# VISION-SJTU/UniDefense

Measured on AMD Instinct MI355X. Metric: images/sec fwd+bwd (256x256, EffNet-b4), higher is better.
Workload: dtype f32

## Files before the change

### include/unidefense_hip.h

```cpp
#ifndef UNIDEFENSE_HIP_H
#define UNIDEFENSE_HIP_H
#include <stdint.h>

#ifdef __cplusplus
extern "C" {
#endif

#define UD_EINVAL (-1000)

typedef void* ud_stream_t;

typedef struct {
    int N, Hin, Win, Cin, Hout, Wout, KH, KW, stride, pad_t, pad_l, transposed;
} ud_conv_geom;

typedef struct {
    const float* A; const float* B; float* C;
    int M, N, K;
    long lda, ldb, ldc;
    int a_mode, b_mode, out_mode, split_k;
    int batch; long strideA, strideB, strideC;
    ud_conv_geom g;
    double* stat_sum; double* stat_sumsq;
    int half_mask;
// ... 126 lines not shown
                  ud_stream_t stream);
int ud_absdiff(const float* a, const float* b, float* out, long total, ud_stream_t stream);

int ud_pix_to_planes(const float* in, float* out, int N, int C, int HW, int mode, ud_stream_t stream);
int ud_planes_to_pix(const float* in, const float* aux, float* out, int N, int C, int HW, int mode,
                     ud_stream_t stream);
int ud_bilinear_fwd(const float* x, float* y, int P, int Hi, int Wi, int Ho, int Wo, ud_stream_t stream);
int ud_bilinear_bwd(const float* dy, float* dx, int P, int Hi, int Wi, int Ho, int Wo, ud_stream_t stream);
int ud_l1_chunks(long per_sample);
int ud_l1_fwd(const float* a, const float* b, float* part, float* out, int N, long per_sample, float scale,
              ud_stream_t stream);
int ud_l1_bwd(const float* a, const float* b, const float* g, float scale, int accumulate, float* da, int N,
              long per_sample, ud_stream_t stream);

int ud_dynfilter_fwd(const float* proj, const float* diff, const float* w2, const float* x, float* pre,
                     int* argmax, float* mask, float* out, int M, int C, int D, int Cx, ud_stream_t stream);
int ud_dynfilter_bwd(const float* dout, const float* dmask_ext, const float* x, const float* mask,
                     const int* argmax, const float* w2, float* dx, float* dlogit, float* dproj, int M,
                     int C, int Cx, ud_stream_t stream);

int ud_avgpool_fwd(const float* x, float* y, int N, int Ho, int Wo, int C, int k, ud_stream_t stream);
int ud_avgpool_bwd(const float* dy, float* dx, int N, int Ho, int Wo, int C, int k, ud_stream_t stream);
int ud_adaptive_avgpool_fwd(const float* x, float* y, int N, int H, int W, int Ho, int Wo, int C, ud_stream_t stream);
int ud_adaptive_avgpool_bwd(const float* dy, float* dx, int N, int H, int W, int Ho, int Wo, int C, ud_stream_t stream);
int ud_maxpool3s2_fwd(const float* x, float* y, unsigned char* arg, int N, int H, int W, int C,
                      ud_stream_t stream);
int ud_maxpool3s2_bwd(const float* dy, const unsigned char* arg, float* dx, int N, int H, int W, int C,
                      ud_stream_t stream);
int ud_add_act_fwd(const float* a, const float* b, int act, float* y, long total, ud_stream_t stream);
int ud_relu_bwd(const float* dy, const float* y, float* g, long total, ud_stream_t stream);
int ud_copy_cols(float* narrow, float* wide, long M, int Cn, int Cw, int off, int dir, ud_stream_t stream);

int ud_aw_triplet(const float* feat, int N, int D, int n_real, float* loss, float* dfeat, float* ws,
                  ud_stream_t stream);

typedef struct {
    const float* feat[3]; float* dfeat[3]; int D[3]; int nfeat;
    const float* cls; const long long* tgt; float* dcls; int N, C, R, F;
    const float* fm; float* dfm; int nfm; const float* sm; float* dsm; int nsm;
    const float* spatial; float* dspatial; const float* freq; float* dfreq;
    float w_cls, w_fm, w_sm, w_trip, w_rec, w_freq;
    float* vals;
    float* ws;
} ud_loss_tail;
int ud_loss_tail_ws_floats(int N, int n_real, int nfeat);
int ud_loss_tail_run(const ud_loss_tail* t, ud_stream_t stream);

int ud_conv_small_supported(int Cin, int Cout, int KH, int KW);
int ud_conv_small(const ud_conv_geom* g, const float* x, const float* wmat, float* y, int Cout, ud_stream_t stream);
int ud_conv_small_wgrad_supported(int Cin, int Ma, int KH, int KW);
long ud_conv_small_wgrad_ws_floats(int Cin, int Ma);
int ud_conv_small_wgrad(const ud_conv_geom* g, const float* a, const float* x, float* part, float* out, int Ma,
                        ud_stream_t stream);

int ud_stem_dgrad_supported(int Cin, int Cout, int KH, int KW, int stride);
int ud_stem_dgrad(const ud_conv_geom* g, const float* dy, const float* w, float* dx, int Cout, int accumulate,
                  ud_stream_t stream);
int ud_absdiff_bwd(const float* a, const float* b, const float* g, float* da, float* db, long total, ud_stream_t stream);
int ud_outer(const float* u, const float* v, float* out, long M, int D, ud_stream_t stream);

int ud_gather2d(const float* in, float* out, const int* iy, const int* ix, long planes, int H, int W,
                ud_stream_t stream);
int ud_blur5_reflect(const float* in, float* out, long planes, int H, int W, float k0, float k1, float k2,
                     ud_stream_t stream);
int ud_amp_mix(const float* A, const float* B, const float* lmda, float* out, long planes, int S, int Whp,
               int planes_per_sample, ud_stream_t stream);
long ud_efdm_ws_bytes(int rows, int L);
int ud_efdm(const float* content, const float* style, const float* lmda, float* out, int rows, int L,
            int rows_per_sample, void* ws, long ws_bytes, ud_stream_t stream);
int ud_coral_moments(const float* x, double* part, int N, int HW, int chunks, ud_stream_t stream);
int ud_affine3(const float* x, const float* M, float* out, int N, int HW, ud_stream_t stream);

typedef struct {
    const double* sum;
    const double* sumsq;
    const float* gamma;
    const float* beta;
    double inv_count;
    double unbias;
    float eps;
    float momentum;
    int act;
    int G;
    float* running_mean;
    float* running_var;
} ud_bn_ref;

long ud_fused_reduce_ws_doubles(int G, int R, int C, int per_group, int min_rows);
int ud_colstats(const void* x, int G, int R, int C, double* sum, double* sumsq, double* ws, int f16, ud_stream_t
    stream);
int ud_colsum_bn(const void* x, const ud_bn_ref* bn, int G, int R, int C, double* out, double* ws, int f16,
    ud_stream_t stream);
int ud_coldot_bn(const void* dy, const void* x, const ud_bn_ref* bn, int G, int R, int C, double* out, double*
    ws, int f16, ud_stream_t stream);
int ud_fc_fwd_d(const double* xsum, float xscale, const float* W, const float* b, float* y, int N, int I, int O,
                ud_stream_t stream);
int ud_se_scale_bn(const void* x, const ud_bn_ref* bn, const float* s, void* y, int G, int R, int C, int f16,
    uint32_t* absmax, ud_stream_t stream);
int ud_colsum_bn_amax(const void* x, const ud_bn_ref* bn, int G, int R, int C, double* out, double* ws, uint32_t* absmax,
                      ud_stream_t stream);
int ud_se_scale_bn_planes(const void* x, const ud_bn_ref* bn, const float* s, uint16_t* planes, long panel_stride,
                          long plane_stride, float* inv_scale, const uint32_t* amax_in, int G, int R, int C,
                          ud_stream_t stream);
int ud_se_scale_bn_plane_half(const void* x, const ud_bn_ref* bn, const float* s, uint16_t* plane, long panel_stride,
                              float* inv_scale, int G, int R, int C, ud_stream_t stream);
int ud_residual_bn(const void* x, const ud_bn_ref* bn, const float* keep, float inv_keep, const void* skip,
// ... 135 lines not shown
```

### unidefense_amd/config.py

```python
import os
from dataclasses import dataclass, fields
from typing import Optional


def _flag(name, default):
    return os.environ.get(name, "1" if default else "0") == "1"


@dataclass
class Config:
    deterministic: bool = False
    fused_mbconv: bool = True
    half_storage: bool = False
    gemm_tune: bool = True
    gemm_tune_defaults: bool = True
    gemm_tune_cache: Optional[str] = None
    engine_graph: bool = True
    syncbn_exchange: bool = True
    force_collectives: bool = False
    hip_adamw: bool = True
    lib_path: Optional[str] = None
    spectral_p2: str = "auto"
    weight_plane_batch: bool = True
    side_branch: bool = False
    expand_bwd_fused: bool = True
    project_bwd_fused: bool = True
    project_bwd_fused_wide: bool = True
    project_fused_narrow: bool = False

    @classmethod
    def from_env(cls):
        c = cls()
        for f in fields(cls):
            env = "UD_" + f.name.upper()
            if f.type is bool:
                setattr(c, f.name, _flag(env, f.default))
            else:
                setattr(c, f.name, os.environ.get(env) or f.default)
        if c.spectral_p2 not in ("auto", "on", "off"):
            raise ValueError(f"UD_SPECTRAL_P2 must be auto, on or off, got {c.spectral_p2!r}")
        return c

    def describe(self):
        return {f.name: getattr(self, f.name) for f in fields(self)}


cfg = Config.from_env()


class override:

    def __init__(self, **kw):
        self.kw, self.saved = kw, {}

    def __enter__(self):
        for k, v in self.kw.items():
            if not hasattr(cfg, k):
                raise AttributeError(k)
            self.saved[k] = getattr(cfg, k)
            setattr(cfg, k, v)
        return cfg

    def __exit__(self, *exc):
        for k, v in self.saved.items():
            setattr(cfg, k, v)
        return False
```

### unidefense_amd/kernels.py

```python
import ctypes as C
import math
import os

import torch

from . import lib as _lib
from .config import cfg as CFG
from .lib import ConvGeom, GemmDesc, GemmP3Desc

_call = _lib.call

GEMM_PROFILE = None


def _stream():
    return C.c_void_p(torch.cuda.current_stream().cuda_stream)


_BR = 0


class branch:
    def __init__(self, b):
        self.b = b
# ... 1136 lines not shown
    key = (Ci, Co, KH, KW)
    if key not in _CONV_SMALL_OK:
        _CONV_SMALL_OK[key] = _call("ud_conv_small_supported", Ci, Co, KH, KW) == 1
    return _CONV_SMALL_OK[key]


_CONV_SMALL_WS = {}
_CONV_SMALL_WGRAD_OK = {}


def _conv_small_wgrad_supported(Ci, Ma, KH, KW):
    key = (Ci, Ma, KH, KW)
    if key not in _CONV_SMALL_WGRAD_OK:
        _CONV_SMALL_WGRAD_OK[key] = _call("ud_conv_small_wgrad_supported", Ci, Ma, KH, KW) == 1
    return _CONV_SMALL_WGRAD_OK[key]


def conv_gather_nt(x, wmat, g):
    _chk(x, wmat)
    M = g.N * g.Hout * g.Wout
    K = g.KH * g.KW * g.Cin
    Co = wmat.shape[0]
    assert wmat.shape[1] == K and x.numel() == g.N * g.Hin * g.Win * g.Cin
    if _CONV_SMALL and M >= _CONV_SMALL_MIN_M and _conv_small_supported(g.Cin, Co, g.KH, g.KW):
        out = empty((g.N, g.Hout, g.Wout, Co), x)
        _call("ud_conv_small", C.byref(g), _p(x), _p(wmat), _p(out), Co, _stream())
        return out
    split = _fwd_split(M, Co, K) if _CONV_SPLITK else 1
    if g.Cin % 4 == 0:
        gk = (g.Hin, g.Win, g.Cin, g.KH, g.KW, g.stride, g.transposed)
        tmp = []

        def scratch():
            if not tmp:
                tmp.append(empty((M, Co), x))
            return tmp[0]
        tuned = _tuned_plan(("conv",) + gk, M, Co, K,
                            lambda cfg, sp: _gemm(x, wmat, scratch(), M, Co, K, 0, K, Co, 2, 0, 2 if sp > 1 else 0, sp, geom=g, cfg=cfg),
                            lambda: _gemm(x, wmat, scratch(), M, Co, K, 0, K, Co, 2, 0, 2 if split > 1 else 0, split, geom=g))
        if tuned is not None:
            cfg, sp = tuned
            out = (split_out if sp > 1 else empty)((g.N, g.Hout, g.Wout, Co), x)
            _gemm(x, wmat, out, M, Co, K, 0, K, Co, 2, 0, 2 if sp > 1 else 0, sp, geom=g, cfg=cfg)
            return out
    if split > 1:
        out = split_out((g.N, g.Hout, g.Wout, Co), x)
        _gemm(x, wmat, out, M, Co, K, 0, K, Co, 2, 0, 2, split, geom=g)
        return out
    out = empty((g.N, g.Hout, g.Wout, Co), x)
    _gemm(x, wmat, out, M, Co, K, 0, K, Co, 2, 0, geom=g)
    return out


_STEM_DGRAD_OK = {}


def stem_dgrad_supported(Ci, Co, KH, KW, stride):
    key = (Ci, Co, KH, KW, stride)
    if key not in _STEM_DGRAD_OK:
        _STEM_DGRAD_OK[key] = _call("ud_stem_dgrad_supported", Ci, Co, KH, KW, stride) == 1
    return _STEM_DGRAD_OK[key]


def stem_dgrad(dy, w, g, out=None):
    Co = w.shape[0]
    if not stem_dgrad_supported(g.Cin, Co, g.KH, g.KW, g.stride):
        raise ValueError(f"no stem data-gradient kernel for Cin {g.Cin}, Cout {Co}, {g.KH}x{g.KW} / {g.stride}")
    dy = dy.contiguous()
    w = w.contiguous()
    _chk(dy, w, out)
    assert dy.numel() == g.N * g.Hout * g.Wout * Co and w.numel() == Co * 3 * g.KH * g.KW and dy.data_ptr() % 16 == 0
    acc = out is not None
    if acc:
        assert out.is_contiguous() and out.dtype == torch.float32 and out.numel() == g.N * 3 * g.Hin * g.Win
    else:
        out = empty((g.N, 3, g.Hin, g.Win), dy)
    _call("ud_stem_dgrad", C.byref(g), _p(dy), _p(w), _p(out), Co, 1 if acc else 0, _stream())
    return out


def absdiff_bwd(a, b, g):
    _chk(a, b, g)
    db = torch.empty_like(b)
    _call("ud_absdiff_bwd", _p(a), _p(b), _p(g), None, _p(db), b.numel(), _stream())
    return db


def outer(u, v):
    _chk(u, v)
    M, D = u.numel(), v.numel()
    out = empty((M, D), u)
    _call("ud_outer", _p(u), _p(v), _p(out), M, D, _stream())
    return out


def conv_gather_wgrad(a, x, g):
    _chk(a, x)
    Kdim = g.N * g.Hout * g.Wout
    Ma = a.shape[-1]
    assert a.numel() == Kdim * Ma
    Ncols = g.KH * g.KW * g.Cin
    if _CONV_SMALL and Kdim >= _CONV_SMALL_MIN_M and _conv_small_wgrad_supported(g.Cin, Ma, g.KH, g.KW):
        need = _call("ud_conv_small_wgrad_ws_floats", g.Cin, Ma)
        ws = _CONV_SMALL_WS.get(_key(a))
        if ws is None or ws.numel() < need:
            ws = _CONV_SMALL_WS[_key(a)] = empty((need,), a)
# ... 1563 lines not shown
```

### unidefense_amd/lib.py

```python
import ctypes as C
import os

_HERE = os.path.dirname(os.path.abspath(__file__))
from .config import cfg as _cfg

LIB_PATH = _cfg.lib_path or os.path.join(_HERE, "libunidefense_hip.so")


class UDLibraryError(RuntimeError):
    pass


class ConvGeom(C.Structure):
    _fields_ = [(n, C.c_int) for n in ("N", "Hin", "Win", "Cin", "Hout", "Wout", "KH", "KW", "stride",
                                       "pad_t", "pad_l", "transposed")]


class GemmDesc(C.Structure):
    _fields_ = [("A", C.c_void_p), ("B", C.c_void_p), ("C", C.c_void_p),
                ("M", C.c_int), ("N", C.c_int), ("K", C.c_int),
                ("lda", C.c_long), ("ldb", C.c_long), ("ldc", C.c_long),
                ("a_mode", C.c_int), ("b_mode", C.c_int), ("out_mode", C.c_int), ("split_k", C.c_int),
                ("batch", C.c_int), ("strideA", C.c_long), ("strideB", C.c_long), ("strideC", C.c_long),
                ("g", ConvGeom), ("stat_sum", C.c_void_p), ("stat_sumsq", C.c_void_p), ("half_mask", C.c_int), ("tile_cfg", C.c_int), ("slice_stride", C.c_long)]
# ... 75 lines not shown
    "ud_norm_bwd_fused": [_P, _P, _I, _I, _I, _P, _P, _P, _P, _I, _P, _P, _P, _P, _P, _P, _P, _P],
    "ud_norm_bwd_apply": [_P, _P, _I, _I, _I, _P, _P, _P, _P, _P, _P, _F, _I, _P, _P],
    "ud_group_colsum": [_P, _I, _I, _I, _F, _P, _P, _P],
    "ud_group_coldot": [_P, _P, _I, _I, _I, _F, _P, _P, _P],
    "ud_dwconv_fwd": [_P, _P, _P] + [_I] * 10 + [_I, _P],
    "ud_dwconv_bwd_data": [_P, _P, _P, _P] + [_I] * 10 + [_I, _P],
    "ud_dw_weights_tapmajor": [_P, _I, _L, _P, _P],
    "ud_dwconv_bwd_weight_parts": [_I, _I],
    "ud_dwconv_bwd_weight": [_P, _P, _P, _P, _I] + [_I] * 10 + [_P],
    "ud_rfft2": [_P, _P, _I, _I, _I, _F, _F, _I, _P],
    "ud_irfft2": [_P, _P, _I, _I, _I, _F, _F, _I, _P],
    "ud_fc_fwd": [_P, _P, _P, _P, _I, _I, _I, _I, _P],
    "ud_fc_bwd": [_P, _P, _P, _P, _P, _P, _I, _I, _I, _I, _P],
    "ud_se_scale_fwd": [_P, _P, _P, _I, _I, _I, _P],
    "ud_se_scale_bwd": [_P, _P, _P, _P, _I, _I, _I, _P],
    "ud_sigmoid_grad_mul": [_P, _P, _L, _P],
    "ud_sfmix_blocks": [_I, _I, _I, _I],
    "ud_sfmix_fwd": [_P, _P, _P, _P, _I, _I, _I, _I, _I, _I, _P],
    "ud_sfmix_bwd": [_P, _P, _P, _P, _P, _P, _P, _P, _I, _I, _I, _I, _I, _I, _P],
    "ud_gate_mix_blocks": [_L],
    "ud_gate_mix_fwd": [_P, _P, _P, _P, _L, _P],
    "ud_gate_mix_bwd": [_P, _P, _P, _P, _P, _P, _P, _P, _L, _P],
    "ud_residual_fwd": [_P, _P, _P, _F, _P, _L, _L, _P],
    "ud_axpby": [_P, _F, _P, _F, _P, _L, _I, _P],
    "ud_mask_scale": [_P, _P, _F, _P, _L, _P],
    "ud_absdiff": [_P, _P, _P, _L, _P],
    "ud_bcast_rows": [_P, _F, _P, _I, _I, _I, _P],
    "ud_pix_to_planes": [_P, _P, _I, _I, _I, _I, _P],
    "ud_planes_to_pix": [_P, _P, _P, _I, _I, _I, _I, _P],
    "ud_bilinear_fwd": [_P, _P, _I, _I, _I, _I, _I, _P],
    "ud_bilinear_bwd": [_P, _P, _I, _I, _I, _I, _I, _P],
    "ud_l1_chunks": [_L],
    "ud_l1_fwd": [_P, _P, _P, _P, _I, _L, _F, _P],
    "ud_l1_bwd": [_P, _P, _P, _F, _I, _P, _I, _L, _P],
    "ud_dynfilter_fwd": [_P, _P, _P, _P, _P, _P, _P, _P, _I, _I, _I, _I, _P],
    "ud_dynfilter_bwd": [_P, _P, _P, _P, _P, _P, _P, _P, _P, _I, _I, _I, _P],
    "ud_avgpool_fwd": [_P, _P, _I, _I, _I, _I, _I, _P],
    "ud_avgpool_bwd": [_P, _P, _I, _I, _I, _I, _I, _P],
    "ud_adaptive_avgpool_fwd": [_P, _P, _I, _I, _I, _I, _I, _I, _P],
    "ud_adaptive_avgpool_bwd": [_P, _P, _I, _I, _I, _I, _I, _I, _P],
    "ud_maxpool3s2_fwd": [_P, _P, _P, _I, _I, _I, _I, _P],
    "ud_maxpool3s2_bwd": [_P, _P, _P, _I, _I, _I, _I, _P],
    "ud_add_act_fwd": [_P, _P, _I, _P, _L, _P],
    "ud_relu_bwd": [_P, _P, _P, _L, _P],
    "ud_copy_cols": [_P, _P, _L, _I, _I, _I, _I, _P],
    "ud_aw_triplet": [_P, _I, _I, _I, _P, _P, _P, _P],
    "ud_loss_tail_ws_floats": [_I, _I, _I],
    "ud_loss_tail_run": [C.POINTER(LossTail), _P],
    "ud_conv_small_supported": [_I, _I, _I, _I],
    "ud_conv_small": [C.POINTER(ConvGeom), _P, _P, _P, _I, _P],
    "ud_conv_small_wgrad_supported": [_I, _I, _I, _I],
    "ud_conv_small_wgrad_ws_floats": [_I, _I],
    "ud_conv_small_wgrad": [C.POINTER(ConvGeom), _P, _P, _P, _P, _I, _P],
    "ud_stem_dgrad_supported": [_I, _I, _I, _I, _I],
    "ud_stem_dgrad": [C.POINTER(ConvGeom), _P, _P, _P, _I, _I, _P],
    "ud_absdiff_bwd": [_P, _P, _P, _P, _P, _L, _P],
    "ud_outer": [_P, _P, _P, _L, _I, _P],
    "ud_gather2d": [_P, _P, _P, _P, _L, _I, _I, _P],
    "ud_blur5_reflect": [_P, _P, _L, _I, _I, _F, _F, _F, _P],
    "ud_amp_mix": [_P, _P, _P, _P, _L, _I, _I, _I, _P],
    "ud_efdm_ws_bytes": [_I, _I],
    "ud_efdm": [_P, _P, _P, _P, _I, _I, _I, _P, _L, _P],
    "ud_coral_moments": [_P, _P, _I, _I, _I, _P],
    "ud_affine3": [_P, _P, _P, _I, _I, _P],
    "ud_fused_reduce_ws_doubles": [_I, _I, _I, _I, _I],
    "ud_colstats": [_P, _I, _I, _I, _P, _P, _P, _I, _P],
    "ud_colsum_bn": [_P, _BN, _I, _I, _I, _P, _P, _I, _P],
    "ud_coldot_bn": [_P, _P, _BN, _I, _I, _I, _P, _P, _I, _P],
    "ud_fc_fwd_d": [_P, _F, _P, _P, _P, _I, _I, _I, _P],
    "ud_se_scale_bn": [_P, _BN, _P, _P, _I, _I, _I, _I, _P, _P],
    "ud_colsum_bn_amax": [_P, _BN, _I, _I, _I, _P, _P, _P, _P],
    "ud_se_scale_bn_plane_half": [_P, _BN, _P, _P, _L, _P, _I, _I, _I, _P],
    "ud_se_scale_bn_planes": [_P, _BN, _P, _P, _L, _L, _P, _P, _I, _I, _I, _P],
    "ud_residual_bn": [_P, _BN, _P, _F, _P, _P, _I, _I, _I, _I, _P, _P],
    "ud_residual_bn_planes": [_P, _BN, _P, _F, _P, _P, _P, _P, _L, _L, _P, _I, _I, _I, _P, _P],
    "ud_normbwd_sums": [_P, _P, _P, _F, _BN, _I, _I, _I, _I, _P, _P, _P, _P, _I, _P],
    "ud_normbwd_apply_plane_half": [_P, _P, _P, _F, _BN, _I, _P, _P, _P, _P, _I, _I, _I, _P, _L, _P, _P, _P, _P],
    "ud_normbwd_apply_planes": [_P, _P, _P, _F, _BN, _I, _P, _P, _P, _P, _P, _I, _I, _I, _P, _L, _L, _P, _P, _P, _P],
    "ud_normbwd_apply": [_P, _P, _P, _F, _BN, _I, _P, _P, _P, _P, _I, _I, _I, _P, _P, _P, _I, _P, _P],
    "ud_pj_bwd_fused_ok": [_I, _I, _I],
    "ud_pj_bwd_fused_grid": [_I, _I, _I, _I],
    "ud_pj_fwd_fused_ok": [_I, _I, _I],
    "ud_pj_fwd_fused": [_P, _BN, _P, _P, _I, _I, _I, _I, _P, _P, _P, _P],
    "ud_pj_bwd_fused_a": [_P, _P, _BN, _P, _P, _I, _I, _I, _I, _P, _P, _P, _P],
    "ud_pj_bwd_fused_b": [_P, _P, _BN, _P, _P, _F, _P, _I, _I, _I, _I, _P, _P, _P, _P],
    "ud_mb_eval_dw_ok": [_I, _I, _I, _I],
    "ud_mb_eval_dw_tiles": [_I, _I, _I],
    "ud_mb_eval_dw": [_P, _P, _BN, _P, _BN, _P, _P] + [_I] * 12 + [_P],
    "ud_mb_eval_dw_h_ok": [_I, _I, _I, _I],
    "ud_mb_eval_dw_h_tiles": [_I, _I, _I],
    "ud_mb_eval_dw_h": [_P, _P, _BN, _P, _BN, _P, _P] + [_I] * 12 + [_P],
    "ud_pw_bwd_fused_ok": [_I, _I],
    "ud_pw_bwd_fused_grid": [_L],
    "ud_pw_bwd_set_form": [_I],
    "ud_pw_bwd_fused": [_P, _P, _BN, _P, _P, _P, _P, _P, _P, _P, _L, _I, _I, _P, _P, _P, _P, _P, _P],
    "ud_normbwd_apply_mix": [_P, _P, _BN, _P, _P, _P, _P, _P, _I, _I, _I, _P, _P, _P, _P, _P, _I, _P],
    "ud_gate_grad_from_acc": [_P, _P, _P, _P],
    "ud_se_bwd_a": [_P, _P, _P, _P, _P, _P, _P, _I, _I, _I, _P],
    "ud_se_bwd_b": [_P, _P, _P, _P, _F, _P, _P, _P, _I, _I, _I, _P],
    "ud_se_scale_bwd_bn": [_P, _P, _BN, _P, _P, _F, _P, _P, _P, _P, _I, _I, _I, _I, _P],
    "ud_bn_apply": [_P, _BN, _P, _I, _I, _I, _I, _P],
    "ud_dwconv_bwd_data_bn": [_P, _P, _I, _P, _P, _P, _BN, _P, _P, _P, _P] + [_I] * 10 + [_I, _P],
    "ud_dwconv_bwd_data_bn_ws_doubles": [_I, _I, _I, _I, _I],
    "ud_dwconv_bwd_data_ex": [_P, _P, _I, _P, _P, _P] + [_I] * 10 + [_I, _P],
    "ud_dwconv_bwd_weight_ex": [_P, _P, _P, _I, _P, _P, _I] + [_I] * 10 + [_I, _P],
    "ud_rfft2_ex": [_P, _P, _I, _I, _I, _F, _F, _BN, _P, _P, _I, _P, _P, _I, _P, _P],
    "ud_rfft2_ex_planes": [_P, _P, _L, _L, _P, _F, _P, _I, _I, _I, _F, _F, _BN, _P, _P, _I, _P, _P, _P, _P, _I, _P],
    "ud_irfft2_mix": [_P, _P, _I, _I, _I, _F, _F, _P, _P, _P, _P, _P, _I, _P],
    "ud_rfft2_two_pass": [_P, _P, _P, _I, _I, _I, _F, _F, _BN, _P, _P, _I, _P, _P, _I, _P, _P],
    "ud_irfft2_two_pass": [_P, _P, _P, _I, _I, _I, _F, _F, _P, _P, _P, _P, _P, _I, _P],
    "ud_fft2_two_pass_ws_floats": [_I, _I, _I],
    "ud_dwtile_ws_doubles": [_I, _I, _I, _I],
    "ud_dwtile": [_P, _BN, _P, _P] + [_I] * 10 + [_P, _I, _P, _P, _BN, _I, _P, _P, _P, _I, _I, _P],
    "ud_dwtile_wgrad_part_rows": [_I, _I, _I],
    "ud_dwtile_wgrad": [_P, _BN, _P, _P, _I, _P, _P, _L] + [_I] * 9 + [_I, _I, _P],
    "ud_dwtile_wgrad_finalize": [_P, _I, _I, _I, _P, _I, _P, _P],
    "ud_dwtile_wgrad_finalize_multi": [C.POINTER(WgradFold), _I, _P],
    "ud_rfft2_ex_plane_half": [_P, _P, _L, _P, _I, _I, _I, _F, _F, _BN, _P, _P, _I, _P, _P, _P, _P, _I, _P],
    "ud_irfft2_dwbwd": [_P, _I, _I, _I, _F, _F, _P, _P, _BN, _P, _I, _P, _I, _P, _P, _P, _P, _P, _P, _I, _P],
    "ud_dwtile_bwd": [_P, _P, _BN, _P, _P, _I, _P, _P, _P, _P, _L, _P, _P, _P] + [_I] * 8 + [_P],
    "ud_rfft2_planes_ws_floats": [_L, _I],
    "ud_rfft2_planes": [_P, _P, _P, _L, _I, _F, _P],
    "ud_rfft2_planes_adjoint": [_P, _P, _P, _L, _I, _F, _P],
    "ud_adamw_chunk_elems": [],
    "ud_adamw_multi": [_P, _P, _I, _P, _P, _I, C.c_double, C.c_double, C.c_double, _I, _I, _P, _P, _P, _P, _P],
    "ud_multi_add": [_P, _P, _P, _I, _P],
    "ud_gemm_get_path": [],
    "ud_sum_slices": [_P, _P, _I, _L, _L, _I, _P],
    "ud_xchg_bytes": [_I, _I, _I],
    "ud_xchg_create": [_I, _I, _I, _P, _P],
    "ud_xchg_open": [_P, _P],
    "ud_xchg_close": [_P],
    "ud_xchg_destroy": [_P],
    "ud_xchg_allreduce": [_P, _I, _P, _I, _I, _I, _I, _P, _P, _L, _P, _P],
}

_COUNT_FUNCS = {"ud_mb_eval_dw_ok", "ud_mb_eval_dw_tiles", "ud_mb_eval_dw_h_ok", "ud_mb_eval_dw_h_tiles", "ud_pj_fwd_fused_ok", "ud_pj_bwd_fused_ok", "ud_pj_bwd_fused_grid", "ud_pw_bwd_fused_ok", "ud_pw_bwd_fused_grid", "ud_loss_tail_ws_floats", "ud_norm_fused_ws_doubles", "ud_norm_fused_counters", "ud_dwtile_wgrad", "ud_dwtile_bwd", "ud_fft32_set_wave", "ud_fft2_two_pass_ws_floats", "ud_dwtile_ws_doubles", "ud_dwtile_wgrad_part_rows", "ud_reduce_ws_doubles", "ud_gemm_query_path", "ud_gemm_get_path", "ud_gemm_stats_slots", "ud_adamw_chunk_elems", "ud_rfft2_planes_ws_floats", "ud_fused_reduce_ws_doubles", "ud_dwconv_bwd_data_bn_ws_doubles", "ud_dwconv_bwd_weight_parts", "ud_sfmix_blocks", "ud_gate_mix_blocks",
                "ud_l1_chunks", "ud_efdm_ws_bytes", "ud_conv_small_supported", "ud_conv_small_wgrad_supported",
                "ud_conv_small_wgrad_ws_floats", "ud_xchg_bytes", "ud_stem_dgrad_supported"}
_LONG_FUNCS = {"ud_mb_eval_dw_tiles", "ud_mb_eval_dw_h_tiles", "ud_pj_bwd_fused_grid", "ud_pw_bwd_fused_grid", "ud_norm_fused_ws_doubles", "ud_fft2_two_pass_ws_floats", "ud_dwtile_ws_doubles", "ud_dwtile_wgrad_part_rows", "ud_xchg_bytes", "ud_efdm_ws_bytes", "ud_rfft2_planes_ws_floats", "ud_conv_small_wgrad_ws_floats", "ud_fused_reduce_ws_doubles",
               "ud_dwconv_bwd_data_bn_ws_doubles"}

EXPORTED = tuple(_SIGNATURES)

_lib = None


def load():
    global _lib
    if _lib is not None:
        return _lib
    if not os.path.exists(LIB_PATH):
        raise UDLibraryError(
            f"{LIB_PATH} is missing: build it with `python -c 'import __graft_entry__ as g; g.build()'` "
            "or `make -C unidefense_amd/csrc`. unidefense_amd has no fallback path.")
    import torch
    if torch.cuda.is_available():
        torch.cuda.init()
    lib = C.CDLL(LIB_PATH)
    for name, argtypes in _SIGNATURES.items():
        fn = getattr(lib, name, None)
        if fn is None:
            raise UDLibraryError(f"{LIB_PATH} does not export {name}; rebuild it")
        fn.argtypes = argtypes
        fn.restype = C.c_long if name in _LONG_FUNCS else C.c_int
    _lib = lib
    return lib


def check(status: int, name: str):
    if status != 0:
        raise UDLibraryError(f"{name} failed with status {status}"
                             + (" (invalid argument)" if status == -1000 else " (-hipError_t)"))


def call(name: str, *args):
    fn = getattr(load(), name)
    st = fn(*args)
    if name in _COUNT_FUNCS:
        if st < 0:
            check(st, name)
        return st
    check(st, name)
    return 0
```

### unidefense_amd/model/unidefense.py

```python
from typing import List, Optional

import torch
import torch.nn as nn

from .. import kernels as K
from ..config import cfg
from .. import tape as T
from .arch import DELIMITER_DICT, build_arch


class _SFConvParams(nn.Conv2d):

    def __init__(self, channels, k):
        super().__init__(channels, channels, k, groups=channels, bias=False)
        self.freq_conv = nn.Conv2d(channels * 2, channels * 2, kernel_size=1, bias=False)
        self.sf_coef = nn.Parameter(torch.tensor(-10.0))


class _MBConvParams(nn.Module):

    def __init__(self, spec, eps, momentum):
        super().__init__()
        self.spec = spec
        if spec.expand != 1:
# ... 310 lines not shown
        ent = T.DW_WT.get(id(w))
        wt = ent[2] if (ent is not None and ent[0] is w) else w.view(CE, k * k).t().contiguous()
        bn1 = K.EvalBN(blk._bn1, 1)
        w2 = blk._project_conv.weight.view(Co, CE)
        pj = K.project_fwd_fused_ok(x, w2, HW)
        d, pool = K.mb_eval_dw(x, blk._expand_conv.weight.view(CE, Ci), K.EvalBN(blk._bn0, 1), wt, bn1, k, s, pt, pl, Ho, Wo,
                               out_act=not pj)
        s1 = K.fc_fwd(pool, blk._se_reduce.weight.view(sp.cse, CE), blk._se_reduce.bias, 0)
        s2 = K.fc_fwd(s1, blk._se_expand.weight.view(CE, sp.cse), blk._se_expand.bias, 1)
        if pj:
            p, _ = K.project_fwd_fused(d, bn1, s2, w2, N, HW)
        else:
            p = K.gemm_nt(K.se_scale_fwd(d, s2).view(N * HW, CE), w2)
        return K.residual_bn(p.view(N, Ho, Wo, Co), K.EvalBN(blk._bn2, 0), None, 1.0, x if sp.skip else None, N, HW)

    def _blocks(self, tape, x, stage, rng, lazy_in=None):
        start = self.delimiter[stage - 1] if stage > 0 else 0
        end = self.delimiter[stage]
        nblk = len(self.backbone._blocks)
        rate0 = self.arch["drop_connect_rate"]
        fused = rng.get("_fused")
        for idx in range(start, end):
            rate = rate0 * float(idx) / nblk if rate0 else 0.0
            keep = rng["drop_connect"].get(idx) if (self.training and rate) else None
            blk = self.backbone._blocks[idx]
            if fused is not None and (blk.spec.sf_norm is None or K.fft_kernel_size(x.shape[1])):
                pend = self.__dict__.setdefault("_nbt_pending", [])
                pend.extend(b.num_batches_tracked for b in (getattr(blk, "_bn0", None), blk._bn1, blk._bn2)
                            if b is not None and b.num_batches_tracked is not None)
                nxt = self.backbone._blocks[idx + 1] if idx + 1 < end else None
                x = T.mbconv_fused(tape, x, blk, keep, 1.0 - rate, fused["wt"][id(blk._depthwise_conv.weight)],
                                   fused["dp"], lazy_in if idx == 0 else None, next_blk=nxt)
            elif rng.get("_eval16") is not None and (blk.spec.sf_norm is None or K.fft_kernel_size(x.shape[1])):
                x = T.mbconv_eval_half(x, blk, rng["_eval16"][id(blk._depthwise_conv.weight)], lazy_in if idx == start else None,
                                       self.EVAL_NODE_H_MAX_CIN)
            elif tape is None and not self.training and self.__dict__.get("_eval_fused") and self._eval_block_ok(blk):
                x = self._mbconv_eval(x, blk)
            else:
                dt = x.dtype
                if dt != torch.float32:
                    x = T.cast(tape, x, torch.float32)
                x = self._mbconv(tape, x, blk, keep, 1.0 - rate)
                if dt != torch.float32:
                    x = T.cast(tape, x, dt)
        return x

    def _sync_group(self, bn):
        group = getattr(self, "_sync_bn_group", None)
        if group is None and isinstance(bn, nn.SyncBatchNorm) and torch.distributed.is_initialized():
            group = bn.process_group or torch.distributed.group.WORLD
        return group

    def _decoder(self, tape, x, dec, last):
        x = T.bias_add(tape, T.conv_dense(tape, x, dec[0].weight, 1, 1, 1, x.shape[1], x.shape[2]), dec[0].bias)
        x = T.instancenorm_act(tape, x, dec[1].weight, dec[1].bias, dec[1].eps, 1)
        x = T.bias_add(tape, T.conv_transpose_s2(tape, x, dec[3].weight), dec[3].bias)
        x = T.instancenorm_act(tape, x, dec[4].weight, dec[4].bias, dec[4].eps, 1)
        x = T.bias_add(tape, T.conv_dense(tape, x, dec[6].weight, 1, 1, 1, x.shape[1], x.shape[2]), dec[6].bias)
        x = T.instancenorm_act(tape, x, dec[7].weight, dec[7].bias, dec[7].eps, 1)
        if last:
            x = T.bias_add(tape, T.conv_dense(tape, x, dec[9].weight, 1, 1, 1, x.shape[1], x.shape[2]), dec[9].bias)
        return x

    def _attention(self, tape, pred_planes, x_planes, emb, rng):
        N, h, w, Cc = emb.shape
        norm = self.freq_norm
        freq_diff, spat_diff, dg = T.attention_diffs(tape, pred_planes, x_planes, h, w, norm)
        emb_freq = T.rfft2_cat(tape, emb, norm)
        ff = self.freq_filter
        proj = T.bias_add(tape, T.conv1x1(tape, emb_freq, ff.layer1[0].weight), ff.layer1[0].bias)
        proj = self._bn(tape, proj, ff.layer1[1], 1)
        f_out, freq_mask = T.dynamic_filter(tape, emb_freq, proj, freq_diff, ff.layer2[0].weight, ff.layer2[0].bias, dg)
        freq_filtered = T.irfft2_split(tape, f_out, norm)

        sfm = self.spat_filter
        proj = T.bias_add(tape, T.conv_dense(tape, emb, sfm.layer1[0].weight, 1, 1, 1, h, w), sfm.layer1[0].bias)
        proj = self._bn(tape, proj, sfm.layer1[1], 1)
        s_out, spat_mask = T.dynamic_filter(tape, emb, proj, spat_diff, sfm.layer2[0].weight, sfm.layer2[0].bias, dg)

        out = T.gate_mix(tape, s_out, freq_filtered, self.fuse_coef)
        e = emb
        if self.training and self.drop_rate > 0:
            e = T.dropout_mask(tape, emb, self._keep_mask(rng, "emb_keep", emb, 1.0 - self.drop_rate), self.drop_rate)
        out = T.add(tape, out, e)
        return out, freq_mask, spat_mask

    @staticmethod
    def _to_pix_mask(m):
        return m.permute(0, 2, 3, 1).contiguous() if m.dim() == 4 else m.contiguous()

    def _prepare_rng(self, rng, n, device):
        out = {"drop_connect": {}, "_given": rng or {}}
        if not self.training:
            return out
        rate0 = self.arch["drop_connect_rate"]
        nblk = len(self.arch["blocks"])
        given = out["_given"].get("drop_connect", {})
        todo = [(idx, rate0 * float(idx) / nblk) for idx, b in enumerate(self.arch["blocks"])
                if b.skip and rate0 and idx > 0]
        fresh = None
        if any(given.get(idx) is None for idx, _ in todo):
            cache = self.__dict__.setdefault("_dc_keep_p", {})
            keep_p = cache.get((device, n))
            if keep_p is None:
                if torch.cuda.is_current_stream_capturing():
                    raise RuntimeError("drop-connect probabilities for a new batch size inside a graph capture: run one eager "
                                       "step with this shape first (the engine and bench.py do)")
                keep_p = cache[(device, n)] = torch.tensor([1.0 - r for _, r in todo], device=device).view(-1, 1).expand(-1, n).contiguous()
            fresh = torch.bernoulli(keep_p)
        for j, (idx, rate) in enumerate(todo):
            k_ = given.get(idx)
# ... 88 lines not shown
```

### unidefense_amd/tape.py

```python
import math
from typing import Optional

import torch

from . import kernels as K
from .config import cfg


class Tape:

    def __init__(self):
        self.nodes = []
        self.grads = {}
        self.param_grads = {}
        self._keep = []
        self.watch = None
        self.captured = {}
        self.kinks = None
        self.gate_cond = {}
        self.param_ready = None
        self.param_uses = None
        self.param_seen = {}
        self._deferred = set()
        self.weight_snapshot = None
# ... 205 lines not shown

    def bwd():
        dy = tape.pop_grad(y)
        if dy is None:
            return
        dy2 = dy.reshape(-1, Co)
        if not _wgrad(tape):
            if need_dx:
                tape.add_grad(x, K.spectral_dgrad(ctx, dy2).view(x.shape))
        elif need_dx:
            dx, dw = K.spectral_bwd(ctx, dy2)
            tape.add_param_grad(w, dw)
            tape.add_grad(x, dx.view(x.shape))
        else:
            tape.wgrad(w, lambda: K.spectral_wgrad(ctx, dy2), dy2)
    tape.record(bwd)
    return y


def _conv_im2col(tape, x, w, wmat, g, need_dx):
    Co, Ci, KH, KW = w.shape
    xcol = K.im2col_planes(x, g)
    y2, ctx = K.spectral_fwd(xcol, wmat, force=True)
    y = y2.view(g.N, g.Hout, g.Wout, Co)
    if _needs(tape):
        def bwd():
            dy = tape.pop_grad(y)
            if dy is None:
                return
            dy2 = dy.reshape(-1, Co)
            if not dy2.is_contiguous():
                dy2 = dy2.contiguous()
            if not _wgrad(tape):
                dcol, dw = (K.spectral_dgrad(ctx, dy2) if need_dx else None), None
            elif need_dx:
                dcol, dw = K.spectral_bwd(ctx, dy2)
            else:
                dcol, dw = None, K.spectral_wgrad(ctx, dy2)
            if dw is not None:
                tape.add_param_grad(w, dw.view(Co, KH, KW, Ci).permute(0, 3, 1, 2).contiguous())
            if need_dx:
                tape.add_grad(x, K.col2im(dcol, g))
        tape.record(bwd)
    return y


def _stem_dgrad(tape, dy, w, g, x_planes):
    cur = tape.grads.pop(id(x_planes), None)
    if cur is not None and not (cur.is_contiguous() and cur.dtype == torch.float32 and cur.shape == x_planes.shape):
        tape.grads[id(x_planes)], cur = cur, None
    tape.add_grad(x_planes, K.stem_dgrad(dy, w, g, out=cur))


def conv_dense(tape, x, w, stride, pad_t, pad_l, Hout, Wout, need_dx=True, x_planes=None):
    N, Hin, Win, Ci = x.shape
    Co, _, KH, KW = w.shape
    g = K.conv_geom(N, Hin, Win, Ci, Hout, Wout, KH, KW, stride, pad_t, pad_l, 0)
    wmat = K.weight_layout(w, 0)
    stem_dx = _tracks(tape, x_planes)
    if K.conv_im2col_ok(g, Co, x):
        assert not stem_dx
        return _conv_im2col(tape, x, w, wmat, g, need_dx)
    y = K.conv_gather_nt(x, wmat, g)
    if _needs(tape):
        wd = K.weight_layout(w, 1) if need_dx else None

        def bwd():
            dy = tape.pop_grad(y)
            if dy is None:
                return
            if need_dx:
                assert stride == 1 and Hout == Hin and Wout == Win, "data gradient implemented for stride 1 'same'"
                gd = K.conv_geom(N, Hout, Wout, Co, Hin, Win, KH, KW, 1, KH - 1 - pad_t, KW - 1 - pad_l, 0)
                tape.add_grad(x, K.conv_gather_nt(dy, wd, gd))
            elif stem_dx:
                _stem_dgrad(tape, dy, w, g, x_planes)
            if _wgrad(tape):
                dw = K.conv_gather_wgrad(dy.view(-1, Co), x, g)
                tape.add_param_grad(w, dw.view(Co, KH, KW, Ci).permute(0, 3, 1, 2).contiguous())
        tape.record(bwd)
    return y


def conv_transpose_s2(tape, x, w):
    N, H, W, Ci = x.shape
    _, Co, KH, KW = w.shape
    Ho, Wo = 2 * H, 2 * W
    g = K.conv_geom(N, H, W, Ci, Ho, Wo, KH, KW, 2, 1, 1, 1)
    wmat = K.weight_layout(w, 2)
    y = K.conv_gather_nt(x, wmat, g)
    if _needs(tape):
        wd = K.weight_layout(w, 0)

        def bwd():
            dy = tape.pop_grad(y)
            if dy is None:
                return
            gd = K.conv_geom(N, Ho, Wo, Co, H, W, KH, KW, 2, 1, 1, 0)
            tape.add_grad(x, K.conv_gather_nt(dy, wd, gd))
            if _wgrad(tape):
                dw = K.conv_gather_wgrad(x.view(-1, Ci), dy, gd)
                tape.add_param_grad(w, dw.view(Ci, KH, KW, Co).permute(0, 3, 1, 2).contiguous())
        tape.record(bwd)
    return y


def linear(tape, x, w, b):
    y = K.fc_fwd(x, w, b, 0)
    if _needs(tape):
        def bwd():
            dy = tape.pop_grad(y)
            if dy is None:
                return
            wg = _wgrad(tape)
            dx, dW, db = K.fc_bwd(dy, w, x, 0, need_dw=wg)
            tape.add_grad(x, dx)
            if wg:
                tape.add_param_grad(w, dW)
                tape.add_param_grad(b, db)
        tape.record(bwd)
    return y


_DW_FUSED_ADD = True
_DW_TILED = True


# ... 1055 lines not shown
```

Measured before the change: 1351.

## Add direct 3x3 decoder conv kernel using split-bf16 MFMA

Adds a dedicated HIP kernel for stride-1 same-padded 3x3 convolutions in the decoder. It stages a halo input tile and the weights in shared memory, splits each fp32 value into three bf16 parts, and accumulates with 16x16x32 bf16 MFMA, using six products per pair to keep close to fp32 accuracy. The kernel replaces the generic gather GEMM for the decoder's forward pass and for its data-gradient pass when the problem is large enough. This removes implicit-GEMM gather overhead, at the cost of six MFMAs per product and a small change in numerics compared with true fp32.

```diff
diff --git a/include/unidefense_hip.h b/include/unidefense_hip.h
--- a/include/unidefense_hip.h
+++ b/include/unidefense_hip.h
@@ -202,6 +202,9 @@
 long ud_conv_small_wgrad_ws_floats(int Cin, int Ma);
 int ud_conv_small_wgrad(const ud_conv_geom* g, const float* a, const float* x, float* part, float* out, int Ma,
                         ud_stream_t stream);
+
+int ud_decconv3x3_supported(const ud_conv_geom* g, int Cout);
+int ud_decconv3x3(const ud_conv_geom* g, const float* x, const float* wmat, float* y, int Cout, ud_stream_t stream);
 
 int ud_stem_dgrad_supported(int Cin, int Cout, int KH, int KW, int stride);
 int ud_stem_dgrad(const ud_conv_geom* g, const float* dy, const float* w, float* dx, int Cout, int accumulate,
diff --git a/unidefense_amd/config.py b/unidefense_amd/config.py
--- a/unidefense_amd/config.py
+++ b/unidefense_amd/config.py
@@ -27,6 +27,7 @@
     project_bwd_fused: bool = True
     project_bwd_fused_wide: bool = True
     project_fused_narrow: bool = False
+    decoder_direct_conv: bool = True
 
     @classmethod
     def from_env(cls):
diff --git a/unidefense_amd/csrc/decconv.hip b/unidefense_amd/csrc/decconv.hip
--- /dev/null
+++ b/unidefense_amd/csrc/decconv.hip
@@ -0,0 +1,182 @@
+#include "ud_common.h"
+
+namespace {
+
+constexpr int NTHREADS = 256;
+constexpr int TW = 16;
+constexpr int HW = TW + 2;
+constexpr int KG = 12;
+
+typedef __bf16 bf16x2 __attribute__((ext_vector_type(2)));
+typedef __bf16 bf16x8 __attribute__((ext_vector_type(8)));
+typedef uint32_t u32x4 __attribute__((ext_vector_type(4)));
+
+__device__ __forceinline__ uint32_t pack_bf16(float x, float y) {
+    bf16x2 v = {(__bf16)x, (__bf16)y};
+    return __builtin_bit_cast(uint32_t, v);
+}
+
+__device__ __forceinline__ void split2(float x, float y, uint32_t& p0, uint32_t& p1, uint32_t& p2) {
+    p0 = pack_bf16(x, y);
+    float rx = x - __uint_as_float(p0 << 16), ry = y - __uint_as_float(p0 & 0xffff0000u);
+    p1 = pack_bf16(rx, ry);
+    float sx = rx - __uint_as_float(p1 << 16), sy = ry - __uint_as_float(p1 & 0xffff0000u);
+    p2 = pack_bf16(sx, sy);
+}
+
+__device__ __forceinline__ void stage8(const float* p, bool ok, int c0, int lim, char* dst, int plane_bytes) {
+    f32x4 v0 = {0.f, 0.f, 0.f, 0.f}, v1 = {0.f, 0.f, 0.f, 0.f};
+    if (ok && c0 < lim) v0 = *reinterpret_cast<const f32x4*>(p);
+    if (ok && c0 + 4 < lim) v1 = *reinterpret_cast<const f32x4*>(p + 4);
+    uint32_t a0, a1, a2, b0, b1, b2, c0_, c1_, c2_, d0, d1, d2;
+    split2(v0[0], v0[1], a0, a1, a2);
+    split2(v0[2], v0[3], b0, b1, b2);
+    split2(v1[0], v1[1], c0_, c1_, c2_);
+    split2(v1[2], v1[3], d0, d1, d2);
+    *reinterpret_cast<u32x4*>(dst) = u32x4{a0, b0, c0_, d0};
+    *reinterpret_cast<u32x4*>(dst + plane_bytes) = u32x4{a1, b1, c1_, d1};
+    *reinterpret_cast<u32x4*>(dst + 2 * plane_bytes) = u32x4{a2, b2, c2_, d2};
+}
+
+template <int MT, int NT>
+__global__ __launch_bounds__(NTHREADS) void decconv3x3_kernel(const float* __restrict__ x, const float* __restrict__ wmat,
+                                                              float* __restrict__ y, int H, int W, int Cin, int Cout) {
+    constexpr int TH = 4 * MT;
+    constexpr int COP = NT * 16;
+    constexpr int A_ITEMS = (TH + 2) * HW;
+    constexpr int B_ITEMS = KG * COP;
+    constexpr int PA = A_ITEMS * 16;
+    constexpr int PB = B_ITEMS * 16;
+    __shared__ __attribute__((aligned(16))) char As[3 * PA];
+    __shared__ __attribute__((aligned(16))) char Bs[3 * PB];
+
+    const int tid = threadIdx.x, lane = tid & 63, wave = tid >> 6;
+    const int l15 = lane & 15, q = lane >> 4;
+    const int ow0 = blockIdx.x * TW, oh0 = blockIdx.y * TH, n = blockIdx.z;
+    const float* xn = x + (long)n * H * W * Cin;
+    const int K9 = 9 * Cin;
+
+    int aoff[3], boff[3];
+#pragma unroll
+    for (int s = 0; s < 3; ++s) {
+        const int tap = 4 * s + q;
+        const int t = tap < 9 ? tap : 0;
+        const int kh = t / 3, kw = t - 3 * kh;
+        aoff[s] = ((wave * MT + kh) * HW + l15 + kw) * 16;
+        boff[s] = (tap * COP + l15) * 16;
+    }
+
+    f32x4 acc[MT][NT];
+#pragma unroll
+    for (int i = 0; i < MT; ++i)
+#pragma unroll
+        for (int j = 0; j < NT; ++j) acc[i][j] = f32x4{0.f, 0.f, 0.f, 0.f};
+
+    for (int c0 = 0; c0 < Cin; c0 += 8) {
+        __syncthreads();
+        for (int it = tid; it < A_ITEMS; it += NTHREADS) {
+            const int r = it / HW, c = it - r * HW;
+            const int ih = oh0 - 1 + r, iw = ow0 - 1 + c;
+            const bool ok = ih >= 0 && ih < H && iw >= 0 && iw < W;
+            const float* p = xn + ((long)(ok ? ih : 0) * W + (ok ? iw : 0)) * Cin + c0;
+            stage8(p, ok, c0, Cin, As + it * 16, PA);
+        }
+        for (int it = tid; it < B_ITEMS; it += NTHREADS) {
+            const int tap = it / COP, co = it - tap * COP;
+            const bool ok = tap < 9 && co < Cout;
+            const float* p = wmat + (long)(ok ? co : 0) * K9 + (ok ? tap : 0) * Cin + c0;
+            stage8(p, ok, c0, Cin, Bs + it * 16, PB);
+        }
+        __syncthreads();
+#pragma unroll
+        for (int s = 0; s < 3; ++s) {
+            bf16x8 fa[MT][3];
+#pragma unroll
+            for (int i = 0; i < MT; ++i)
+#pragma unroll
+                for (int p = 0; p < 3; ++p)
+                    fa[i][p] = *reinterpret_cast<const bf16x8*>(As + p * PA + aoff[s] + i * HW * 16);
+#pragma unroll
+            for (int j = 0; j < NT; ++j) {
+                bf16x8 fb[3];
+#pragma unroll
+                for (int p = 0; p < 3; ++p) fb[p] = *reinterpret_cast<const bf16x8*>(Bs + p * PB + boff[s] + j * 256);
+#pragma unroll
+                for (int i = 0; i < MT; ++i) {
+                    f32x4 c = acc[i][j];
+                    c = __builtin_amdgcn_mfma_f32_16x16x32_bf16(fa[i][2], fb[0], c, 0, 0, 0);
+                    c = __builtin_amdgcn_mfma_f32_16x16x32_bf16(fa[i][0], fb[2], c, 0, 0, 0);
+                    c = __builtin_amdgcn_mfma_f32_16x16x32_bf16(fa[i][1], fb[1], c, 0, 0, 0);
+                    c = __builtin_amdgcn_mfma_f32_16x16x32_bf16(fa[i][1], fb[0], c, 0, 0, 0);
+                    c = __builtin_amdgcn_mfma_f32_16x16x32_bf16(fa[i][0], fb[1], c, 0, 0, 0);
+                    c = __builtin_amdgcn_mfma_f32_16x16x32_bf16(fa[i][0], fb[0], c, 0, 0, 0);
+                    acc[i][j] = c;
+                }
+            }
+        }
+    }
+
+#pragma unroll
+    for (int i = 0; i < MT; ++i) {
+        const int oh = oh0 + wave * MT + i;
+        if (oh >= H) continue;
+        float* yr = y + (((long)n * H + oh) * W + ow0 + 4 * q) * Cout;
+#pragma unroll
+        for (int j = 0; j < NT; ++j) {
+            const int co = j * 16 + l15;
+            if (co < Cout) {
+#pragma unroll
+                for (int r = 0; r < 4; ++r) yr[(long)r * Cout + co] = acc[i][j][r];
+            }
+        }
+    }
+}
+
+template <int MT, int NT>
+int launch(const ud_conv_geom& g, const float* x, const float* wmat, float* y, int Cout, hipStream_t s) {
+    dim3 grid((unsigned)(g.Wout / TW), (unsigned)ud_cdiv(g.Hout, 4 * MT), (unsigned)g.N);
+    hipLaunchKernelGGL((decconv3x3_kernel<MT, NT>), grid, dim3(NTHREADS), 0, s, x, wmat, y, g.Hout, g.Wout, g.Cin, Cout);
+    UD_LAUNCH_CHECK();
+    return 0;
+}
+
+int pick_mt(const ud_conv_geom& g) {
+    const long segs = (long)g.N * g.Hout * (g.Wout / TW);
+    if (segs / 16 >= 512) return 4;
+    if (segs / 8 >= 512) return 2;
+    return 1;
+}
+
+template <int NT>
+int launch_nt(const ud_conv_geom& g, const float* x, const float* wmat, float* y, int Cout, hipStream_t s) {
+    switch (pick_mt(g)) {
+        case 4: return launch<4, NT>(g, x, wmat, y, Cout, s);
+        case 2: return launch<2, NT>(g, x, wmat, y, Cout, s);
+        default: return launch<1, NT>(g, x, wmat, y, Cout, s);
+    }
+}
+
+}
+
+extern "C" {
+
+int ud_decconv3x3_supported(const ud_conv_geom* g, int Cout) {
+    if (!g) return 0;
+    if (g->KH != 3 || g->KW != 3 || g->stride != 1 || g->pad_t != 1 || g->pad_l != 1 || g->transposed) return 0;
+    if (g->Hout != g->Hin || g->Wout != g->Win || g->Wout % TW != 0 || g->Hout < 1 || g->N < 1) return 0;
+    if (g->Cin < 4 || g->Cin % 4 != 0 || Cout < 1 || Cout > 160) return 0;
+    return 1;
+}
+
+int ud_decconv3x3(const ud_conv_geom* g, const float* x, const float* wmat, float* y, int Cout, ud_stream_t stream) {
+    if (!ud_decconv3x3_supported(g, Cout)) return UD_EINVAL;
+    if (((uintptr_t)x | (uintptr_t)wmat) & 15) return UD_EINVAL;
+    hipStream_t s = (hipStream_t)stream;
+    const int nt = (Cout + 15) / 16;
+    if (nt <= 2) return launch_nt<2>(*g, x, wmat, y, Cout, s);
+    if (nt <= 3) return launch_nt<3>(*g, x, wmat, y, Cout, s);
+    if (nt <= 5) return launch_nt<5>(*g, x, wmat, y, Cout, s);
+    return launch_nt<10>(*g, x, wmat, y, Cout, s);
+}
+
+}
diff --git a/unidefense_amd/kernels.py b/unidefense_amd/kernels.py
--- a/unidefense_amd/kernels.py
+++ b/unidefense_amd/kernels.py
@@ -1212,6 +1212,32 @@
     return out
 
 
+_DECCONV_OK = {}
+
+
+def decconv3x3_ok(x, Co, g):
+    key = (g.N, g.Hin, g.Win, g.Cin, g.Hout, g.Wout, g.KH, g.KW, g.stride, g.pad_t, g.pad_l, g.transposed, Co)
+    if key not in _DECCONV_OK:
+        _DECCONV_OK[key] = _call("ud_decconv3x3_supported", C.byref(g), Co) == 1
+    return _DECCONV_OK[key] and x.dtype == torch.float32 and x.is_contiguous() and x.data_ptr() % 16 == 0
+
+
+_DECCONV_MIN_M = 16384
+
+
+def decconv3x3_wanted(x, Co, g):
+    return g.N * g.Hout * g.Wout >= _DECCONV_MIN_M and decconv3x3_ok(x, Co, g)
+
+
+def decconv3x3(x, wmat, g):
+    _chk(x, wmat)
+    Co = wmat.shape[0]
+    assert wmat.shape[1] == 9 * g.Cin and x.numel() == g.N * g.Hin * g.Win * g.Cin and wmat.is_contiguous()
+    out = empty((g.N, g.Hout, g.Wout, Co), x)
+    _call("ud_decconv3x3", C.byref(g), _p(x), _p(wmat), _p(out), Co, _stream())
+    return out
+
+
 _STEM_DGRAD_OK = {}
 
 
diff --git a/unidefense_amd/lib.py b/unidefense_amd/lib.py
--- a/unidefense_amd/lib.py
+++ b/unidefense_amd/lib.py
@@ -151,6 +151,8 @@
     "ud_conv_small_wgrad_supported": [_I, _I, _I, _I],
     "ud_conv_small_wgrad_ws_floats": [_I, _I],
     "ud_conv_small_wgrad": [C.POINTER(ConvGeom), _P, _P, _P, _P, _I, _P],
+    "ud_decconv3x3_supported": [C.POINTER(ConvGeom), _I],
+    "ud_decconv3x3": [C.POINTER(ConvGeom), _P, _P, _P, _I, _P],
     "ud_stem_dgrad_supported": [_I, _I, _I, _I, _I],
     "ud_stem_dgrad": [C.POINTER(ConvGeom), _P, _P, _P, _I, _I, _P],
     "ud_absdiff_bwd": [_P, _P, _P, _P, _P, _L, _P],
@@ -236,7 +238,8 @@
 
 _COUNT_FUNCS = {"ud_mb_eval_dw_ok", "ud_mb_eval_dw_tiles", "ud_mb_eval_dw_h_ok", "ud_mb_eval_dw_h_tiles", "ud_pj_fwd_fused_ok", "ud_pj_bwd_fused_ok", "ud_pj_bwd_fused_grid", "ud_pw_bwd_fused_ok", "ud_pw_bwd_fused_grid", "ud_loss_tail_ws_floats", "ud_norm_fused_ws_doubles", "ud_norm_fused_counters", "ud_dwtile_wgrad", "ud_dwtile_bwd", "ud_fft32_set_wave", "ud_fft2_two_pass_ws_floats", "ud_dwtile_ws_doubles", "ud_dwtile_wgrad_part_rows", "ud_reduce_ws_doubles", "ud_gemm_query_path", "ud_gemm_get_path", "ud_gemm_stats_slots", "ud_adamw_chunk_elems", "ud_rfft2_planes_ws_floats", "ud_fused_reduce_ws_doubles", "ud_dwconv_bwd_data_bn_ws_doubles", "ud_dwconv_bwd_weight_parts", "ud_sfmix_blocks", "ud_gate_mix_blocks",
                 "ud_l1_chunks", "ud_efdm_ws_bytes", "ud_conv_small_supported", "ud_conv_small_wgrad_supported",
-                "ud_conv_small_wgrad_ws_floats", "ud_xchg_bytes", "ud_stem_dgrad_supported"}
+                "ud_conv_small_wgrad_ws_floats", "ud_xchg_bytes", "ud_stem_dgrad_supported",
+                "ud_decconv3x3_supported"}
 _LONG_FUNCS = {"ud_mb_eval_dw_tiles", "ud_mb_eval_dw_h_tiles", "ud_pj_bwd_fused_grid", "ud_pw_bwd_fused_grid", "ud_norm_fused_ws_doubles", "ud_fft2_two_pass_ws_floats", "ud_dwtile_ws_doubles", "ud_dwtile_wgrad_part_rows", "ud_xchg_bytes", "ud_efdm_ws_bytes", "ud_rfft2_planes_ws_floats", "ud_conv_small_wgrad_ws_floats", "ud_fused_reduce_ws_doubles",
                "ud_dwconv_bwd_data_bn_ws_doubles"}
 
diff --git a/unidefense_amd/model/unidefense.py b/unidefense_amd/model/unidefense.py
--- a/unidefense_amd/model/unidefense.py
+++ b/unidefense_amd/model/unidefense.py
@@ -386,11 +386,12 @@
         return group
 
     def _decoder(self, tape, x, dec, last):
-        x = T.bias_add(tape, T.conv_dense(tape, x, dec[0].weight, 1, 1, 1, x.shape[1], x.shape[2]), dec[0].bias)
+        direct = cfg.decoder_direct_conv
+        x = T.bias_add(tape, T.conv_dense(tape, x, dec[0].weight, 1, 1, 1, x.shape[1], x.shape[2], direct=direct), dec[0].bias)
         x = T.instancenorm_act(tape, x, dec[1].weight, dec[1].bias, dec[1].eps, 1)
         x = T.bias_add(tape, T.conv_transpose_s2(tape, x, dec[3].weight), dec[3].bias)
         x = T.instancenorm_act(tape, x, dec[4].weight, dec[4].bias, dec[4].eps, 1)
-        x = T.bias_add(tape, T.conv_dense(tape, x, dec[6].weight, 1, 1, 1, x.shape[1], x.shape[2]), dec[6].bias)
+        x = T.bias_add(tape, T.conv_dense(tape, x, dec[6].weight, 1, 1, 1, x.shape[1], x.shape[2], direct=direct), dec[6].bias)
         x = T.instancenorm_act(tape, x, dec[7].weight, dec[7].bias, dec[7].eps, 1)
         if last:
             x = T.bias_add(tape, T.conv_dense(tape, x, dec[9].weight, 1, 1, 1, x.shape[1], x.shape[2]), dec[9].bias)
diff --git a/unidefense_amd/tape.py b/unidefense_amd/tape.py
--- a/unidefense_amd/tape.py
+++ b/unidefense_amd/tape.py
@@ -281,7 +281,7 @@
     tape.add_grad(x_planes, K.stem_dgrad(dy, w, g, out=cur))
 
 
-def conv_dense(tape, x, w, stride, pad_t, pad_l, Hout, Wout, need_dx=True, x_planes=None):
+def conv_dense(tape, x, w, stride, pad_t, pad_l, Hout, Wout, need_dx=True, x_planes=None, direct=False):
     N, Hin, Win, Ci = x.shape
     Co, _, KH, KW = w.shape
     g = K.conv_geom(N, Hin, Win, Ci, Hout, Wout, KH, KW, stride, pad_t, pad_l, 0)
@@ -290,7 +290,8 @@
     if K.conv_im2col_ok(g, Co, x):
         assert not stem_dx
         return _conv_im2col(tape, x, w, wmat, g, need_dx)
-    y = K.conv_gather_nt(x, wmat, g)
+    direct = direct and not stem_dx and K.decconv3x3_wanted(x, Co, g)
+    y = K.decconv3x3(x, wmat, g) if direct else K.conv_gather_nt(x, wmat, g)
     if _needs(tape):
         wd = K.weight_layout(w, 1) if need_dx else None
 
@@ -301,7 +302,10 @@
             if need_dx:
                 assert stride == 1 and Hout == Hin and Wout == Win, "data gradient implemented for stride 1 'same'"
                 gd = K.conv_geom(N, Hout, Wout, Co, Hin, Win, KH, KW, 1, KH - 1 - pad_t, KW - 1 - pad_l, 0)
-                tape.add_grad(x, K.conv_gather_nt(dy, wd, gd))
+                if direct and K.decconv3x3_wanted(dy, Ci, gd):
+                    tape.add_grad(x, K.decconv3x3(dy, wd, gd))
+                else:
+                    tape.add_grad(x, K.conv_gather_nt(dy, wd, gd))
             elif stem_dx:
                 _stem_dgrad(tape, dy, w, g, x_planes)
             if _wgrad(tape):
```

Result: no change. 1360 (median of 6 runs) (+0.7%).
